# liuzl/rwkv-tts-rs

Measured on AMD Instinct MI355X. Metric: audio samples/sec (16 kHz) for RWKV-TTS 0.4B, batch=32 per GPU, higher is better.
Workload: dtype bf16; 1 GPU; config3: 32 requests/GPU, P=32 prompt, 32 global + 512 semantic tokens, exact sampler, + BiCodec vocoder -> PCM (vocoder of batch s overlapped with LM of batch s+1 on its own stream); global_batch=32, seq_len=577, parallelism=dp1 (request sharding)

## Files before the change

include/rwkvtts.h:

```cpp
#ifndef RWKVTTS_H
#define RWKVTTS_H

#include <stddef.h>
#include <stdint.h>

#ifdef __cplusplus
extern "C" {
#endif

#define RWKVTTS_EOS_TOKEN 8192
#define RWKVTTS_TAG_0 8193
#define RWKVTTS_TAG_1 8194
#define RWKVTTS_TAG_2 8195
#define RWKVTTS_GLOBAL_TOKEN_OFFSET 8196
#define RWKVTTS_SPECIAL_TOKEN_OFFSET 77823
#define RWKVTTS_N_GLOBAL 32
#define RWKVTTS_SEMANTIC_LIMIT 2048
#define RWKVTTS_HOP 320
#define RWKVTTS_SAMPLE_RATE 16000

#define RWKVTTS_OK 0
#define RWKVTTS_EINVAL -1
#define RWKVTTS_EHIP -2
#define RWKVTTS_ENOMEM -3
// ... 98 lines not shown
  int32_t token_chunk_size;
  int32_t use_graphs;
  int32_t wkv_variant;
  int32_t quant_layers;
  int32_t quant_type;
  uint32_t forms;
} rwkvtts_engine_desc;

#define RWKVTTS_FORM_SEPARATE_ATT 1u
#define RWKVTTS_FORM_SEPARATE_FFN 2u
#define RWKVTTS_FORM_LN_ROWS 4u
#define RWKVTTS_FORM_SLAB_HANDOFF 8u
#define RWKVTTS_FORM_SEPARATE_LNOUT 16u
#define RWKVTTS_FORM_SEPARATE_EMBED 32u
#define RWKVTTS_FORM_EXACT_SAMPLER 64u

#define RWKVTTS_QUANT_NONE 0
#define RWKVTTS_QUANT_INT8 1
#define RWKVTTS_QUANT_NF4 2
#define RWKVTTS_QUANT_SF4 3

int rwkvtts_engine_create(const rwkvtts_engine_desc* desc, const void* weights, size_t bytes,
                          int blob_on_device, rwkvtts_engine** out);
int rwkvtts_engine_destroy(rwkvtts_engine* e);
const char* rwkvtts_last_error(void);
int rwkvtts_engine_dims(const rwkvtts_engine* e, rwkvtts_dims* out);

int64_t rwkvtts_state_floats(const rwkvtts_engine* e);
int rwkvtts_slot_reset(rwkvtts_engine* e, int slot);
int rwkvtts_slot_read(rwkvtts_engine* e, int slot, float* host_out);
// ... 113 lines not shown
  int32_t persistent[RWKVTTS_MAX_ENGINES];
} rwkvtts_manager_stats;
int rwkvtts_manager_get_stats(rwkvtts_manager* m, rwkvtts_manager_stats* out);

typedef struct {
  int64_t steps;
  int64_t prefill_steps;
  double decode_ms;
  double prefill_ms;
  double sample_ms;
  int64_t decode_rows;
  int32_t profile_kernel_count;
  int32_t persistent;
} rwkvtts_stats;
int rwkvtts_get_stats(rwkvtts_engine* e, rwkvtts_stats* out);

int rwkvtts_set_profiling(rwkvtts_engine* e, int on);
int rwkvtts_profile_entry(rwkvtts_engine* e, int idx, char* name, int name_cap, int64_t* launches,
                          double* total_ms);

int rwkvtts_debug_advance(rwkvtts_engine* e, const float* logits, int n_rows, const void* rows, int exact,
                          int n_steps, int32_t* out_tok, int32_t* out_used, int32_t* out_phase);
int rwkvtts_debug_advance_ex(rwkvtts_engine* e, const float* logits, int n_rows, const void* rows, int exact,
                             int n_steps, int32_t* out_tok, int32_t* out_used, int32_t* out_phase);

typedef struct rwkvtts_codec rwkvtts_codec;
typedef struct {
  int32_t codebook_size;
  int32_t codebook_dim;
  int32_t latent_dim;
// ... 197 lines not shown
```

rwkv-tts-rs_amd/csrc/api.cpp:

```cpp
#include <string.h>

#include <mutex>
#include <new>

#include "engine.h"

namespace rwkvtts {
static thread_local std::string g_last_error;
void set_error(const std::string& msg) { g_last_error = msg; }
}

using namespace rwkvtts;

struct rwkvtts_engine {
  std::mutex mu;
  Engine eng;
};
#define LOCK(e) std::lock_guard<std::mutex> lock_((e)->mu)

#define GUARD(body)                                      \
  try {                                                  \
    body                                                 \
  } catch (const std::bad_alloc&) {                      \
    set_error("out of host memory");                     \
// ... 124 lines not shown
        results[i].n_global = results[i].n_semantic = 0;
      }
    return rc;
  })
}

int rwkvtts_get_stats(rwkvtts_engine* e, rwkvtts_stats* out) {
  RT_CHECK(e && out, RWKVTTS_EINVAL, "null argument");
  LOCK(e);
  *out = e->eng.stats;
  out->profile_kernel_count = (int32_t)e->eng.prof.size();
  out->persistent = e->eng.persistent() ? 1 : 0;
  return RWKVTTS_OK;
}

int rwkvtts_set_profiling(rwkvtts_engine* e, int on) {
  RT_CHECK(e, RWKVTTS_EINVAL, "null engine");
  RT_CHECK(on >= 0 && on <= 2, RWKVTTS_EINVAL, "set_profiling: 0, 1 or 2");
  LOCK(e);
  GUARD({
    e->eng.profiling = on == 1;
    return e->eng.set_graph_timing(on == 2);
  })
}

int rwkvtts_profile_entry(rwkvtts_engine* e, int idx, char* name, int name_cap, int64_t* launches,
                          double* total_ms) {
  RT_CHECK(e, RWKVTTS_EINVAL, "null engine");
  LOCK(e);
  RT_CHECK(idx >= 0 && idx < (int)e->eng.prof.size(), RWKVTTS_EINVAL, "profile index out of range");
// ... 12 lines not shown
```

rwkv-tts-rs_amd/csrc/engine.h:

```cpp
#pragma once
#include <map>
#include <string>
#include <vector>

#include "lm_kernels.h"
#include "sampler.h"
#include "sched.h"

namespace rwkvtts {

struct DebugAdvanceRow {
  int32_t mode;
  int32_t phase;
  int32_t top_k;
  int32_t fixed;
  int32_t n_sem;
  int32_t hard_min;
  int32_t win_bits;
  int32_t win_len;
  uint32_t key[8];
  uint64_t draw;
};
struct DebugAdvanceRowEx {
  DebugAdvanceRow row;
// ... 57 lines not shown
             rwkvtts_rng* const* rngs, int32_t* out, float* dbg_host = nullptr);
  int generate(const rwkvtts_request* reqs, int n, rwkvtts_result* res, const rwkvtts_token_sink* sinks = nullptr);
  int debug_advance(const float* logits, int n_rows, const struct DebugAdvanceRow* rows, int exact, int n_steps,
                    int32_t* out_tok, int32_t* out_used, int32_t* out_phase);
  int debug_advance_ex(const float* logits, int n_rows, const struct DebugAdvanceRowEx* rows, int exact, int n_steps,
                       int32_t* out_tok, int32_t* out_used, int32_t* out_phase);
  int serve(JobSource& src);
  bool validate(const rwkvtts_request& q, std::string& why) const { return rwkvtts::validate(q, dims.n_vocab, why); }
  int max_slots() const { return S_; }
  bool persistent() const { return att_persist_ || ffn_persist_; }
  bool take_recovered() {
    const bool r = recovered_;
    recovered_ = false;
    return r;
  }
  int64_t max_active = 0;
  int64_t admissions_ = 0;

  rwkvtts_dims dims{};
  rwkvtts_stats stats{};
  bool profiling = false;
  std::vector<ProfEntry> prof;
  int set_graph_timing(bool on);
  bool graph_timing() const { return d_gt_ != nullptr && gtime_; }

 private:
  int run_step(const StepPlan& p, bool upload);
  struct ServeState;
  struct Unit {
    bool valid = false, prefill = false, uploaded = false;
    int buf = 0;
  };
  int serve_loop(ServeState& st);
  int admit(ServeState& st, Job* j);
  int launch_unit(ServeState& st, Unit& u);
  int enqueue_snapshot(ServeState& st, const Unit& u);
  int finish_unit(const Unit& u, ServeState& st);
  int accumulate_stamps(const Unit& u);
  int launch_forward(int R, int n_seg, int n_lg, int head_rows, bool tok_from_ctrl, bool advance,
                     bool sampling_params = false);
  int upload_plan(const StepPlan& p);
  void prof_begin(hipEvent_t* ev);
  void prof_end(const char* name, hipEvent_t ev);
  int flush_prof();
  int dump_stamps();
  int reset_persistent();
  int degrade_persistent();
  static constexpr int64_t kDegradeWindow = 1024;
  int64_t units_ = 0;
// ... 80 lines not shown
      if ((int)tl_names_.size() > tl_n_) tl_names_.resize(tl_n_);
    }
    return RWKVTTS_OK;
  }
  static constexpr int kTlMax = 1024;
  bf16_t* wpack_ = nullptr;
  bf16_t* lora_pack_ = nullptr;
  const bf16_t* emb_ = nullptr;
  const bf16_t* head_ = nullptr;
  const float *ln0_w_ = nullptr, *ln0_b_ = nullptr, *lnout_w_ = nullptr, *lnout_b_ = nullptr;
  std::vector<LayerW> L_;
  float* wkv_ = nullptr;
  float* att_sh_ = nullptr;
  float* ffn_sh_ = nullptr;
  int* slot_par_ = nullptr;
  std::vector<int> par_host_;
  std::vector<SlotCtrl> ctrl_stage_;
  uint32_t* d_tok_ = nullptr;
  int4* d_rows_ = nullptr;
  int4* d_segs_ = nullptr;
  int* d_lg_rows_ = nullptr;
  int* d_lg_slot_ = nullptr;
  float *h0_ = nullptr, *h1_ = nullptr, *partA_ = nullptr, *partO_ = nullptr, *partF_ = nullptr,
        *partK_ = nullptr,
        *vfirst_ = nullptr, *logits_ = nullptr;
  bf16_t *xm_hi_ = nullptr, *xm_lo_ = nullptr, *z_hi_ = nullptr, *z_lo_ = nullptr,
         *xf_hi_ = nullptr, *xf_lo_ = nullptr, *xk_hi_ = nullptr, *xk_lo_ = nullptr,
         *xo_hi_ = nullptr, *xo_lo_ = nullptr;
  SlotCtrl* d_ctrl_ = nullptr;
  int32_t* d_sem_ = nullptr;
  SlotCtrl* h_ctrl_ = nullptr;
  int32_t* h_prog_ = nullptr;
// ... 28 lines not shown
```

rwkv-tts-rs_amd/csrc/engine.hip:

```cpp
#include "engine.h"

#include <fcntl.h>
#include <string.h>
#include <sys/file.h>
#include <unistd.h>

#include <algorithm>
#include <chrono>
#include <deque>
#include <map>
#include <mutex>
#include <random>

namespace rwkvtts {

template <typename T>
int Engine::alloc(T** p, size_t count) {
  void* q = nullptr;
  RT_HIP(hipMalloc(&q, std::max<size_t>(count * sizeof(T), 256)));
  RT_HIP(hipMemset(q, 0, std::max<size_t>(count * sizeof(T), 256)));
  allocs_.push_back(q);
  *p = (T*)q;
  return RWKVTTS_OK;
}
// ... 50 lines not shown
    if (*lock_fd >= 0) close(*lock_fd);
    *lock_fd = -1;
  }
}

Engine::~Engine() {
  release_persistent(device_, this, &lock_fd_);
  hipSetDevice(device_);
  if (stream_) hipStreamSynchronize(stream_);
  for (auto& g : graphs_) hipGraphExecDestroy(g.second);
  for (auto& e : pending_prof_) hipEventDestroy(e.second);
  for (void* p : allocs_) hipFree(p);
  for (void* p : {(void*)d_samp_logits_, (void*)d_keys_, (void*)d_draws_, (void*)d_out_, d_wide_})
    if (p) hipFree(p);
  if (h_ctrl_) hipHostFree(h_ctrl_);
  if (h_prog_) hipHostFree(h_prog_);
  if (h_gt_) hipHostFree(h_gt_);
  if (stream_) hipStreamDestroy(stream_);
}

#define RT_OK(x)                      \
  do {                                \
    int _r = (x);                     \
    if (_r != RWKVTTS_OK) return _r;  \
  } while (0)

int Engine::init(const rwkvtts_engine_desc& desc, const void* weights, size_t bytes, int on_device) {
  device_ = desc.device;
  RT_HIP(hipSetDevice(device_));
  {
// ... 32 lines not shown
  auto pick = [](int K, int want) {
    int ks = std::max(128, std::min(std::min(want, 512), K));
    while (ks > 128 && K % ks) ks >>= 1;
    return K / ks;
  };
  splitA_ = pick(C, 256);
  splitO_ = pick(C, 128);
  splitK_ = pick(C, 256);
  splitF_ = pick(F, 256);
  splitH_ = pick(C, 512);
  RT_CHECK(C % 128 == 0 && F % 128 == 0, RWKVTTS_EUNSUPPORTED, "K dims must be multiples of 128");
  RT_CHECK(splitA_ <= kMaxParts, RWKVTTS_EUNSUPPORTED, "n_embd too large for the WKV partial sum (raise kMaxParts)");
  state_perm_ = wkv_perm_layout(dims.d_decay, dims.d_aaa, dims.d_mv, dims.d_gate, splitA_, S_, desc.wkv_variant);
  constexpr uint32_t kKnownForms = RWKVTTS_FORM_SEPARATE_ATT | RWKVTTS_FORM_SEPARATE_FFN | RWKVTTS_FORM_LN_ROWS |
                                   RWKVTTS_FORM_SLAB_HANDOFF | RWKVTTS_FORM_SEPARATE_LNOUT |
                                   RWKVTTS_FORM_SEPARATE_EMBED | RWKVTTS_FORM_EXACT_SAMPLER;
  RT_CHECK((desc.forms & ~kKnownForms) == 0, RWKVTTS_EINVAL, "engine desc: unknown forms bits");
  att_persist_ = !(desc.forms & RWKVTTS_FORM_SEPARATE_ATT);
  ffn_persist_ = !(desc.forms & RWKVTTS_FORM_SEPARATE_FFN);
  fuse_ln1_ = !(desc.forms & RWKVTTS_FORM_LN_ROWS);
  gran_ = !(desc.forms & RWKVTTS_FORM_SLAB_HANDOFF);
  lnrow_ = !(desc.forms & RWKVTTS_FORM_SEPARATE_LNOUT);
  no_emb_fuse_ = (desc.forms & RWKVTTS_FORM_SEPARATE_EMBED) != 0;
  exact_sampler_ = (desc.forms & RWKVTTS_FORM_EXACT_SAMPLER) != 0;
  if ((ffn_persist_ || att_persist_) && !claim_persistent(desc.device, this, &lock_fd_)) ffn_persist_ = att_persist_ = false;
  if (const char* ds = getenv("RWKVTTS_DEBUG_STAMPS")) {
    std::string spec(ds);
    size_t pos = 0;
    while (pos < spec.size()) {
      size_t end = spec.find(';', pos);
      if (end == std::string::npos) end = spec.size();
      const std::string item = spec.substr(pos, end - pos);
      pos = end + 1;
      const size_t eq = item.find('=');
      if (eq == std::string::npos) continue;
      const std::string kind = item.substr(0, eq), path = item.substr(eq + 1);
      if (kind == "gemm") {
        dbg_gstamp_path_ = path;
        RT_OK(alloc(&dbg_gstamps_, 2 * 4096 * 4));
// ... 124 lines not shown
    for (int l = 0; l < dims.n_layer; ++l) {
      LayerW& w = L_[l];
      pack(w.wr, C, C, true); pack(w.wk, C, C, true); pack(w.wv, C, C, true);
      pack(w.w1t, Dw, C, true); pack(w.a1t, Da, C, true); pack(w.v1t, Dv, C, true); pack(w.g1t, Dg, C, true);
      pack(w.wo, C, C); pack(w.ffn_k, F, C); pack(w.ffn_v, C, F);
    }
    pack(head_, dims.n_vocab, C);
    RT_HIP(hipGetLastError());
  }
  RT_HIP(hipStreamSynchronize(stream_));
  const int64_t Lc = dims.n_layer;
  RT_OK(alloc(&wkv_, (size_t)S_ * Lc * H_ * 64 * 64));
  RT_OK(alloc(&att_sh_, (size_t)2 * S_ * Lc * C));
  RT_OK(alloc(&ffn_sh_, (size_t)2 * S_ * Lc * C));
  RT_OK(alloc(&slot_par_, (size_t)S_));
  par_host_.assign(S_, 0);
  ctrl_stage_.assign(S_, SlotCtrl{});
  RT_OK(alloc(&d_tok_, (size_t)Rmax_));
  RT_OK(alloc(&d_rows_, (size_t)Rmax_));
  RT_OK(alloc(&d_segs_, (size_t)std::max(Rmax_, S_)));
  RT_OK(alloc(&d_lg_rows_, (size_t)Rmax_));
  RT_OK(alloc(&d_lg_slot_, (size_t)Rmax_));
  const size_t RC = (size_t)Rmax_ * C;
  RT_OK(alloc(&h0_, RC));
  RT_OK(alloc(&h1_, RC));
  RT_OK(alloc(&xm_hi_, 6 * RC));
  RT_OK(alloc(&xm_lo_, 6 * RC));
  RT_OK(alloc(&partA_, (size_t)splitA_ * Rmax_ * ldA_));
  RT_OK(alloc(&z_hi_, RC));
  RT_OK(alloc(&z_lo_, RC));
  RT_OK(alloc(&partO_, (size_t)splitO_ * RC));
  RT_OK(alloc(&xf_hi_, RC));
// ... 31 lines not shown
    sync_bufs_.push_back({(int*)d_gran_, (size_t)ffn_gran_count(4, dims.n_ffn) * sizeof(uint64_t)});
    const int64_t ng = att_gran_count((int)dims.n_embd);
    RT_OK(alloc(&d_gran_att_, (size_t)ng));
    sync_bufs_.push_back({(int*)d_gran_att_, (size_t)ng * sizeof(uint64_t)});
  }

  RT_HIP(hipDeviceSynchronize());
  return RWKVTTS_OK;
}

int64_t Engine::state_floats() const {
  const int64_t C = dims.n_embd;
  return (int64_t)dims.n_layer * (2 * C + (int64_t)H_ * 64 * 64);
}

int Engine::slot_reset(int slot, bool sync) {
  RT_CHECK(slot >= 0 && slot < S_, RWKVTTS_EINVAL, "slot out of range");
  RT_HIP(hipSetDevice(device_));
  const int64_t C = dims.n_embd, Lc = dims.n_layer, per = Lc * H_ * 64 * 64;
  RT_HIP(hipMemsetAsync(wkv_ + slot * per, 0, per * 4, stream_));
  for (int p = 0; p < 2; ++p) {
    RT_HIP(hipMemsetAsync(att_sh_ + ((int64_t)p * S_ + slot) * Lc * C, 0, Lc * C * 4, stream_));
    RT_HIP(hipMemsetAsync(ffn_sh_ + ((int64_t)p * S_ + slot) * Lc * C, 0, Lc * C * 4, stream_));
  }
  par_host_[slot] = 0;
  RT_HIP(hipMemcpyAsync(slot_par_ + slot, &par_host_[slot], 4, hipMemcpyHostToDevice, stream_));
  if (sync) RT_HIP(hipStreamSynchronize(stream_));
  return RWKVTTS_OK;
}

static inline int64_t perm_index(int kind, int i, int j) {
  if (kind == 1) {
    const int t = 2 * i + (j >> 5), q = (j & 31) >> 2, e = j & 3;
    return ((int64_t)q * 128 + t) * 4 + e;
  }
  const int t = 4 * i + (j >> 4), q = (j & 15) >> 2, e = j & 3;
  return ((int64_t)q * 256 + t) * 4 + e;
}
void Engine::state_permute(const float* std_block, float* dev_block) {
  for (int i = 0; i < 64; ++i)
    for (int j = 0; j < 64; ++j) dev_block[perm_index(state_perm_, i, j)] = std_block[i * 64 + j];
}
// ... 15 lines not shown
    RT_HIP(hipMemcpy(o + C, wkv_ + ((int64_t)slot * Lc + l) * HNN, HNN * 4, hipMemcpyDeviceToHost));
    if (state_perm_) {
      std::vector<float> tmp(o + C, o + C + HNN);
      for (int h = 0; h < H_; ++h) state_unpermute(tmp.data() + (int64_t)h * 4096, o + C + (int64_t)h * 4096);
    }
    RT_HIP(hipMemcpy(o + C + HNN, ffn_sh_ + (((int64_t)par * S_ + slot) * Lc + l) * C, C * 4, hipMemcpyDeviceToHost));
  }
  return RWKVTTS_OK;
}

int Engine::slot_write(int slot, const float* in) {
  RT_CHECK(slot >= 0 && slot < S_, RWKVTTS_EINVAL, "slot out of range");
  RT_HIP(hipSetDevice(device_));
  RT_HIP(hipStreamSynchronize(stream_));
  const int64_t C = dims.n_embd, Lc = dims.n_layer, HNN = (int64_t)H_ * 64 * 64;
  par_host_[slot] = 0;
  RT_HIP(hipMemcpy(slot_par_ + slot, &par_host_[slot], 4, hipMemcpyHostToDevice));
  for (int64_t l = 0; l < Lc; ++l) {
    const float* o = in + l * (2 * C + HNN);
    RT_HIP(hipMemcpy(att_sh_ + (((int64_t)0 * S_ + slot) * Lc + l) * C, o, C * 4, hipMemcpyHostToDevice));
    if (state_perm_) {
      std::vector<float> tmp(HNN);
      for (int h = 0; h < H_; ++h) state_permute(o + C + (int64_t)h * 4096, tmp.data() + (int64_t)h * 4096);
      RT_HIP(hipMemcpy(wkv_ + ((int64_t)slot * Lc + l) * HNN, tmp.data(), HNN * 4, hipMemcpyHostToDevice));
    } else {
      RT_HIP(hipMemcpy(wkv_ + ((int64_t)slot * Lc + l) * HNN, o + C, HNN * 4, hipMemcpyHostToDevice));
    }
    RT_HIP(hipMemcpy(ffn_sh_ + (((int64_t)0 * S_ + slot) * Lc + l) * C, o + C + HNN, C * 4, hipMemcpyHostToDevice));
  }
  return RWKVTTS_OK;
}

// ... 705 lines not shown
int Engine::generate(const rwkvtts_request* reqs, int n, rwkvtts_result* res, const rwkvtts_token_sink* sinks) {
  stats = rwkvtts_stats{};
  max_active = 0;
  ListSource src(reqs, n, res, sinks);
  const int rc = serve(src);
  if (rc != RWKVTTS_OK && sinks) src.fail_rest(rc);
  return rc;
}

struct Engine::ServeState {
  explicit ServeState(JobSource& s) : src(s) {}
  JobSource& src;
  std::vector<Active> act;
  std::vector<int> free_slots;
  std::vector<Job*> fresh;
  bool open = true;
  Unit pending;
  StepPlan dp;
  bool dp_valid = false;
  UnitEvents ev;
  std::random_device rd;
};

int Engine::admit(ServeState& st, Job* j) {
  const rwkvtts_request& q = j->req;
  j->res->status = 0;
  j->res->n_global = j->res->n_semantic = 0;
  std::string why;
  if (!validate(q, why)) {
    set_error("request rejected: " + why);
// ... 12 lines not shown
                         hipHostMallocDefault));
  if (const char* fa = getenv("RWKVTTS_TEST_FAIL_ADMIT")) {
    if (++admissions_ == atoi(fa)) {
      set_error("injected admission failure (RWKVTTS_TEST_FAIL_ADMIT)");
      return RWKVTTS_EHIP;
    }
  }
  Admission ad = admission_of(q, q.has_seed ? 0 : (((uint64_t)st.rd() << 32) ^ st.rd()));
  const int slot = st.free_slots.back();
  st.free_slots.pop_back();
  rwkvtts_rng rg, rs;
  rwkvtts_rng_seed_from_u64(ad.gseed, &rg);
  rwkvtts_rng_seed_from_u64(ad.sseed, &rs);
  memcpy(ad.ctrl.gkey, rg.key, 32);
  memcpy(ad.ctrl.skey, rs.key, 32);
  RT_OK(slot_reset(slot, false));
  ctrl_stage_[slot] = ad.ctrl;
  RT_HIP(hipMemcpyAsync(d_ctrl_ + slot, &ctrl_stage_[slot], sizeof(SlotCtrl), hipMemcpyHostToDevice, stream_));
  Active a;
  a.job = j;
  a.slot = slot;
  a.sink = sink_of(j);
  a.zero_shot = ad.zero_shot;
  a.pinned = ad.pinned;
  a.own_sampling = ad.own_sampling;
  a.prompt = std::move(ad.prompt);
  a.total = ad.total;
  st.act.push_back(std::move(a));
  st.dp_valid = false;
  return RWKVTTS_OK;
}

int Engine::launch_unit(ServeState& st, Unit& u) {
  std::vector<Active>& act = st.act;
  u.valid = true;
  u.uploaded = false;
  u.prefill = std::any_of(act.begin(), act.end(), [](const Active& a) { return a.in_prompt(); });
  u.buf = st.pending.valid ? st.pending.buf ^ 1 : 0;
  RT_HIP(hipEventRecord(st.ev.ev0[u.buf], stream_));
  if (u.prefill) {
    RT_OK(run_step(mixed_plan(act, chunk_, dims.n_vocab), true));
    st.dp_valid = false;
    stats.prefill_steps++;
    return RWKVTTS_OK;
  }
  if (!st.dp_valid) {
    st.dp = decode_plan(act);
    RT_OK(upload_plan(st.dp));
    st.dp_valid = u.uploaded = true;
  }
  const int K = window_len(act, kLookahead, profiling || d_tl_);
  if (d_tl_) RT_HIP(hipMemsetAsync(d_tl_, 0, (size_t)kTlStride * kTlMax * 8, stream_));
  for (int k = 0; k < K; ++k) {
    st.dp.head_rows = head_rows_of(act, dims.n_vocab);
    RT_OK(run_step(st.dp, false));
    for (auto& a : act) a.advances++;
// ... 68 lines not shown
    while ((q = hipEventQuery(st.ev.ev1[b])) == hipErrorNotReady) __builtin_ia32_pause();
    RT_HIP(q);
  }
  float ms = 0;
  hipEventElapsedTime(&ms, st.ev.ev0[b], st.ev.ev1[b]);
  (u.prefill ? stats.prefill_ms : stats.decode_ms) += ms;
  RT_OK(flush_prof());
  RT_OK(accumulate_stamps(u));
  ++units_;
  const SlotCtrl* snap = h_ctrl_ + (size_t)b * (S_ + 1);
  if (const int code = *(const int*)(snap + S_)) {
    persist_fault_ = code;
    set_error("persistent decode launch: a hand-off wait timed out (code " + std::to_string(code) + ")");
    return RWKVTTS_EHIP;
  }
  auto retiring = [&](const Active& a) { return !a.in_prompt() && snap[a.slot].phase == kPhDone; };
  bool copied = false;
  for (auto& a : act) {
    const SlotCtrl& c = snap[a.slot];
    if (!retiring(a) || !a.job->res->semantic_tokens || c.n_sem <= 0) continue;
    RT_HIP(hipMemcpyAsync(a.job->res->semantic_tokens, d_sem_ + (int64_t)a.slot * RWKVTTS_SEMANTIC_LIMIT,
                          sizeof(int32_t) * c.n_sem, hipMemcpyDeviceToHost, stream_));
    copied = true;
  }
  if (copied) RT_HIP(hipStreamSynchronize(stream_));
  for (auto& a : act) {
    if (!a.sink || a.in_prompt()) continue;
    const SlotCtrl& c = snap[a.slot];
    const bool done = c.phase == kPhDone;
    const int n = std::min(c.n_sem, a.copied_hi[b]);
// ... 22 lines not shown
    st.free_slots.push_back(act[i].slot);
    act.erase(act.begin() + i);
  }
  if (act.size() != st.dp.rows.size()) st.dp_valid = false;
  return RWKVTTS_OK;
}

int Engine::serve_loop(ServeState& st) {
  while (true) {
    if (st.open && !st.free_slots.empty()) {
      st.open = st.src.next((int)st.free_slots.size(), st.act.empty(), st.fresh);
      while (!st.fresh.empty()) {
        RT_OK(admit(st, st.fresh.front()));
        st.fresh.erase(st.fresh.begin());
      }
    }
    if (st.act.empty()) {
      if (!st.open) return RWKVTTS_OK;
      continue;
    }
    std::sort(st.act.begin(), st.act.end(), [](const Active& x, const Active& y) { return x.slot < y.slot; });
    Unit now;
    RT_OK(launch_unit(st, now));
    RT_OK(enqueue_snapshot(st, now));
    if (st.pending.valid) {
      const Unit old = st.pending;
      st.pending.valid = false;
      RT_OK(finish_unit(old, st));
    }
    const bool can_admit = st.open && !st.free_slots.empty();
// ... 15 lines not shown
    const int code = persist_fault_;
    persist_fault_ = 0;
    const bool degrade = last_fault_unit_ >= 0 && units_ - last_fault_unit_ <= kDegradeWindow;
    last_fault_unit_ = units_;
    recovered_ = reset_persistent() == RWKVTTS_OK && (!degrade || degrade_persistent() == RWKVTTS_OK);
    if (recovered_ && d_drop_ && test_drops_left_ > 0) {
      --test_drops_left_;
      const int one = 1;
      recovered_ = hipMemcpy(d_drop_, &one, sizeof(int), hipMemcpyHostToDevice) == hipSuccess;
    }
    set_error("persistent decode launch: a hand-off wait timed out (code " + std::to_string(code) +
              "); the unit's requests failed, the engine was reset" +
              (degrade ? " and now runs the separate launches (second timeout)" : ""));
  }
  if (rc != RWKVTTS_OK) {
    for (Job* j : st.fresh) fail_job(src, j, rc, 0);
    for (auto& a : st.act) fail_job(src, a.job, rc, a.sink ? a.delivered : -1);
    return rc;
  }
  return dump_stamps();
}

int Engine::reset_persistent() {
  RT_HIP(hipSetDevice(device_));
  RT_HIP(hipMemsetAsync(d_ctrl_ + S_, 0, sizeof(SlotCtrl), stream_));
  for (auto& b : sync_bufs_) RT_HIP(hipMemsetAsync(b.first, 0, b.second, stream_));
  if (d_epoch_) {
    int ep = 0;
    RT_HIP(hipMemcpyAsync(&ep, d_epoch_, sizeof(int), hipMemcpyDeviceToHost, stream_));
    RT_HIP(hipStreamSynchronize(stream_));
// ... 77 lines not shown
```

rwkv-tts-rs_amd/csrc/sched.h:

```cpp
#pragma once
#include <math.h>
#include <stdint.h>
#include <string.h>

#include <algorithm>
#include <string>
#include <vector>

#include "../../include/rwkvtts.h"
#include "slot_ctrl.h"

namespace rwkvtts {

struct Job;

struct alignas(16) Int4 {
  int32_t x, y, z, w;
};

struct StepPlan {
  std::vector<uint32_t> tok;
  std::vector<Int4> rows;
  std::vector<Int4> segs;
  std::vector<int> lg_rows;
// ... 5 lines not shown
};

struct Active {
  Job* job = nullptr;
  int slot = 0;
  std::vector<uint32_t> prompt;
  int prefilled = 0;
  int advances = 0;
  int total = 0;
  bool zero_shot = false;
  bool pinned = false;
  bool own_sampling = false;
  const rwkvtts_token_sink* sink = nullptr;
  int delivered = 0;
  int copied_hi[2] = {0, 0};
  bool in_prompt() const { return prefilled < (int)prompt.size(); }
};

inline bool is_zero_shot(const rwkvtts_request& q) { return q.ref_global != nullptr && q.ref_semantic != nullptr; }
inline bool is_pinned(const rwkvtts_request& q) { return q.pinned_voice != 0; }

inline bool validate(const rwkvtts_request& q, int n_vocab, std::string& why) {
  auto ids_ok = [&](const int32_t* p, int n, int lo, int hi, const char* what) {
    if (n < 0 || (n > 0 && !p)) {
      why = std::string(what) + ": bad array";
      return false;
    }
    for (int i = 0; i < n; ++i)
      if (p[i] < lo || p[i] >= hi) {
        why = std::string(what) + ": id " + std::to_string(p[i]) + " out of range";
// ... 124 lines not shown
    c.phase = kPhSemantic;
    for (int i = 0; i < RWKVTTS_N_GLOBAL; ++i) {
      a.prompt.push_back((uint32_t)(q.ref_global[i] + RWKVTTS_GLOBAL_TOKEN_OFFSET));
      c.global_out[c.n_global++] = q.ref_global[i];
    }
    a.prompt.push_back(RWKVTTS_TAG_1);
    a.total = c.sem_limit;
  } else {
    c.mode = 0;
    c.phase = kPhGlobal;
    a.total = RWKVTTS_N_GLOBAL + 1 + c.sem_limit;
  }
  return a;
}

inline void append_decode_row(StepPlan& p, int slot) {
  const int r = (int)p.rows.size();
  p.rows.push_back({slot, kRowFirst | kRowLast | kRowCtrl, -1, 0});
  if (!p.tok_from_ctrl) p.tok.push_back(0);
  p.segs.push_back({slot, r, 1, 0});
  p.lg_rows.push_back(r);
  p.lg_slot.push_back(slot);
}

enum LogitRows { kLogitsNone, kLogitsLast, kLogitsAll };

inline void append_token_rows(StepPlan& p, int slot, const uint32_t* tok, int take, LogitRows lg) {
  const int r0 = (int)p.rows.size();
  for (int t = 0; t < take; ++t) {
    const int flags = (t == 0 ? kRowFirst : 0) | (t == take - 1 ? kRowLast : 0);
// ... 13 lines not shown
    if (!a.in_prompt()) all_global &= !a.zero_shot && !a.pinned && a.advances <= RWKVTTS_N_GLOBAL;
  return std::min(all_global ? 4096 : 8193, n_vocab);
}

inline StepPlan mixed_plan(std::vector<Active>& act, int chunk, int n_vocab) {
  StepPlan p;
  p.advance = true;
  int budget = chunk;
  for (const Active& a : act) {
    if (a.in_prompt()) continue;
    append_decode_row(p, a.slot);
    --budget;
  }
  budget = std::max(budget, 1);
  for (Active& a : act) {
    const int left = (int)a.prompt.size() - a.prefilled;
    if (left <= 0 || budget <= 0) continue;
    const int take = std::min(left, budget);
    append_token_rows(p, a.slot, a.prompt.data() + a.prefilled, take, take == left ? kLogitsLast : kLogitsNone);
    a.prefilled += take;
    budget -= take;
  }
  p.head_rows = head_rows_of(act, n_vocab);
  p.sampling_params = any_own_sampling(act);
  for (Active& a : act) a.advances += !a.in_prompt();
  return p;
}

inline StepPlan decode_plan(const std::vector<Active>& act) {
  StepPlan p;
  p.tok_from_ctrl = true;
  p.advance = true;
  p.sampling_params = any_own_sampling(act);
  for (const Active& a : act) append_decode_row(p, a.slot);
  return p;
}

inline int window_len(const std::vector<Active>& act, int lookahead, bool single) {
  int K = single ? 1 : lookahead;
  for (const Active& a : act) K = std::min(K, std::max(1, a.total - a.advances));
// ... 19 lines not shown
```

rwkv-tts-rs_amd/rwkvtts/_ffi.py:

```python
import ctypes
import os

_HERE = os.path.dirname(os.path.abspath(__file__))
LIB_PATH = os.environ.get("RWKVTTS_LIB") or os.path.join(_HERE, "librwkvtts.so")


def build_id() -> str:
    import glob
    import hashlib
    csrc = os.path.join(_HERE, "..", "csrc")
    inc = os.path.join(_HERE, "..", "..", "include")
    files = sorted(glob.glob(os.path.join(csrc, "*.hip")) + glob.glob(os.path.join(csrc, "*.cpp")) +
                   glob.glob(os.path.join(csrc, "*.h")) + [os.path.join(csrc, "Makefile")] +
                   glob.glob(os.path.join(inc, "*.h")), key=os.path.basename)
    h = hashlib.sha256()
    for f in files:
        h.update(os.path.basename(f).encode())
        with open(f, "rb") as fh:
            h.update(fh.read())
    return h.hexdigest()[:16]

EOS_TOKEN = 8192
TAG_0, TAG_1, TAG_2 = 8193, 8194, 8195
GLOBAL_TOKEN_OFFSET = 8196
# ... 11 lines not shown

class Dims(ctypes.Structure):
    _fields_ = [(n, ctypes.c_int32) for n in (
        "n_layer", "n_embd", "head_size", "n_ffn", "n_vocab", "d_decay", "d_aaa", "d_mv", "d_gate")]


class EngineDesc(ctypes.Structure):
    _fields_ = [("device", ctypes.c_int32), ("max_slots", ctypes.c_int32),
                ("token_chunk_size", ctypes.c_int32), ("use_graphs", ctypes.c_int32),
                ("wkv_variant", ctypes.c_int32), ("quant_layers", ctypes.c_int32),
                ("quant_type", ctypes.c_int32), ("forms", ctypes.c_uint32)]


FORM_SEPARATE_ATT, FORM_SEPARATE_FFN, FORM_LN_ROWS, FORM_SLAB_HANDOFF = 1, 2, 4, 8
FORM_SEPARATE_LNOUT, FORM_SEPARATE_EMBED, FORM_EXACT_SAMPLER = 16, 32, 64
CODEC_WEIGHTS_AUTO, CODEC_WEIGHTS_BF16, CODEC_WEIGHTS_HILO = 0, 1, 2
CODEC_FORM_SEPARATE_RESUNIT, CODEC_FORM_CHANNEL_LAST = 1, 2


QUANT_NONE, QUANT_INT8, QUANT_NF4, QUANT_SF4 = 0, 1, 2, 3


class Input(ctypes.Structure):
    _fields_ = [("slot", ctypes.c_int32), ("tokens", ctypes.POINTER(ctypes.c_uint32)),
                ("n_tokens", ctypes.c_int32), ("option", ctypes.c_int32)]


class Rng(ctypes.Structure):
    _fields_ = [("key", ctypes.c_uint32 * 8), ("draw_index", ctypes.c_uint64)]

# ... 23 lines not shown
                ("sampling_set", ctypes.c_int32), ("global_sampling", PhaseSampling),
                ("semantic_sampling", PhaseSampling), ("pinned_voice", ctypes.c_int32)]


class Result(ctypes.Structure):
    _fields_ = [("status", ctypes.c_int32), ("n_global", ctypes.c_int32),
                ("n_semantic", ctypes.c_int32), ("global_tokens", ctypes.c_int32 * N_GLOBAL),
                ("semantic_tokens", ctypes.POINTER(ctypes.c_int32))]


class Stats(ctypes.Structure):
    _fields_ = [("steps", ctypes.c_int64), ("prefill_steps", ctypes.c_int64),
                ("decode_ms", ctypes.c_double), ("prefill_ms", ctypes.c_double),
                ("sample_ms", ctypes.c_double), ("decode_rows", ctypes.c_int64),
                ("profile_kernel_count", ctypes.c_int32), ("persistent", ctypes.c_int32)]


class ManagerDesc(ctypes.Structure):
    _fields_ = [("n_engines", ctypes.c_int32), ("devices", ctypes.c_int32 * MAX_ENGINES),
                ("engine", EngineDesc), ("max_batch_size", ctypes.c_int32),
                ("collect_timeout_ms", ctypes.c_int32)]


class ManagerStats(ctypes.Structure):
    _fields_ = [("submitted", ctypes.c_int64), ("completed", ctypes.c_int64), ("batches", ctypes.c_int64),
                ("served", ctypes.c_int64 * MAX_ENGINES), ("max_active", ctypes.c_int64 * MAX_ENGINES),
                ("steps", ctypes.c_int64 * MAX_ENGINES), ("bcast_ranks", ctypes.c_int32),
                ("bcast_rccl", ctypes.c_int32), ("bcast_ms", ctypes.c_double),
                ("waiters", ctypes.c_int32), ("reserved", ctypes.c_int32),
                ("persistent", ctypes.c_int32 * MAX_ENGINES)]
# ... 101 lines not shown
                                                     ctypes.POINTER(ctypes.c_uint64)]),
    "rwkvtts_manager_wait_tokens": (ctypes.c_int, [ctypes.c_void_p, ctypes.c_uint64, ctypes.c_int32, ctypes.c_int,
                                                   ctypes.c_void_p, ctypes.POINTER(ctypes.c_int32), ctypes.c_void_p,
                                                   ctypes.POINTER(ctypes.c_int32), ctypes.POINTER(ctypes.c_int32),
                                                   ctypes.POINTER(ctypes.c_int32)]),
    "rwkvtts_manager_create": (ctypes.c_int, [ctypes.POINTER(ManagerDesc), ctypes.c_void_p, ctypes.c_size_t,
                                              ctypes.POINTER(ctypes.c_void_p)]),
    "rwkvtts_manager_destroy": (ctypes.c_int, [ctypes.c_void_p]),
    "rwkvtts_manager_submit": (ctypes.c_int, [ctypes.c_void_p, ctypes.POINTER(Request),
                                              ctypes.POINTER(ctypes.c_uint64)]),
    "rwkvtts_manager_wait": (ctypes.c_int, [ctypes.c_void_p, ctypes.c_uint64, ctypes.c_int, ctypes.POINTER(Result)]),
    "rwkvtts_manager_generate_batch": (ctypes.c_int, [ctypes.c_void_p, ctypes.POINTER(Request), ctypes.c_int,
                                                      ctypes.POINTER(Result)]),
    "rwkvtts_manager_get_stats": (ctypes.c_int, [ctypes.c_void_p, ctypes.POINTER(ManagerStats)]),
    "rwkvtts_get_stats": (ctypes.c_int, [ctypes.c_void_p, ctypes.POINTER(Stats)]),
    "rwkvtts_set_profiling": (ctypes.c_int, [ctypes.c_void_p, ctypes.c_int]),
    "rwkvtts_debug_advance": (ctypes.c_int, [ctypes.c_void_p, ctypes.c_void_p, ctypes.c_int, ctypes.c_void_p,
                                             ctypes.c_int, ctypes.c_int, ctypes.c_void_p, ctypes.c_void_p,
                                             ctypes.c_void_p]),
    "rwkvtts_debug_advance_ex": (ctypes.c_int, [ctypes.c_void_p, ctypes.c_void_p, ctypes.c_int, ctypes.c_void_p,
                                                ctypes.c_int, ctypes.c_int, ctypes.c_void_p, ctypes.c_void_p,
                                                ctypes.c_void_p]),
    "rwkvtts_profile_entry": (ctypes.c_int, [ctypes.c_void_p, ctypes.c_int, ctypes.c_char_p, ctypes.c_int,
                                             ctypes.POINTER(ctypes.c_int64), ctypes.POINTER(ctypes.c_double)]),
    "rwkvtts_codec_blob_bytes": (ctypes.c_int64, [ctypes.POINTER(CodecDims)]),
    "rwkvtts_codec_synth_weights": (ctypes.c_int, [ctypes.POINTER(CodecDims), ctypes.c_uint64, ctypes.c_void_p]),
    "rwkvtts_codec_create": (ctypes.c_int, [ctypes.c_int, ctypes.POINTER(CodecDims), ctypes.c_void_p,
                                            ctypes.POINTER(ctypes.c_void_p)]),
    "rwkvtts_codec_create_ex": (ctypes.c_int, [ctypes.c_int, ctypes.POINTER(CodecDims), ctypes.c_void_p,
                                               ctypes.c_int, ctypes.POINTER(ctypes.c_void_p)]),
# ... 101 lines not shown
```

rwkv-tts-rs_amd/rwkvtts/runtime.py:

```python
import ctypes
import dataclasses
import threading
from typing import List, Optional, Sequence

import numpy as np

from . import _ffi
from ._ffi import check, lib


class StdRng:

    def __init__(self, rng_struct):
        self._s = rng_struct

    @classmethod
    def seed_from_u64(cls, seed: int) -> "StdRng":
        s = _ffi.Rng()
        lib().rwkvtts_rng_seed_from_u64(ctypes.c_uint64(seed & 0xFFFFFFFFFFFFFFFF), ctypes.byref(s))
        return cls(s)

    @property
    def key(self):
        return list(self._s.key)
# ... 265 lines not shown
                sinks[i].fn = fns[-1]
        rc = lib().rwkvtts_generate_batch_stream(self._h, reqs, n, res, sinks)
        if raised:
            raise raised[0]
        check(rc, "generate_batch_stream")
        out, self.last_status = _unpack_results(res, sem_bufs)
        return out

    @_locked
    def stats(self):
        s = _ffi.Stats()
        check(lib().rwkvtts_get_stats(self._h, ctypes.byref(s)), "get_stats")
        return {f: getattr(s, f) for f, _ in _ffi.Stats._fields_}

    @_locked
    def set_profiling(self, on):
        mode = on if isinstance(on, int) and not isinstance(on, bool) else (1 if on else 0)
        check(lib().rwkvtts_set_profiling(self._h, mode), "set_profiling")

    @_locked
    def profile(self):
        out = {}
        n = self.stats()["profile_kernel_count"]
        for i in range(n):
            name = ctypes.create_string_buffer(64)
            la = ctypes.c_int64()
            ms = ctypes.c_double()
            check(lib().rwkvtts_profile_entry(self._h, i, name, 64, ctypes.byref(la), ctypes.byref(ms)), "profile_entry")
            out[name.value.decode()] = (int(la.value), float(ms.value))
        return out
# ... 246 lines not shown
```

Before: 11.12 million samples/s.

## Add prompt prefix state cache and batched slot admission kernel

Adds an 8-entry cache of recurrent state keyed on the property-token prefix of each request. A hit restores the WKV and shift state in a single admission kernel and skips prefilling those tokens. A miss makes the request build the entry, with the prefill split so the state can be snapshotted at the prefix boundary and then published. Per-slot memsets and control copies are replaced by one batched k_admit launch per admission round. The trade-off is an extra tail prefill step and publish copies on misses, plus device memory for the cache entries.

Result: slower. 10.99 million samples/s (-1.2%).

```diff
diff --git a/include/rwkvtts.h b/include/rwkvtts.h
--- a/include/rwkvtts.h
+++ b/include/rwkvtts.h
@@ -136,6 +136,7 @@
 #define RWKVTTS_FORM_SEPARATE_LNOUT 16u
 #define RWKVTTS_FORM_SEPARATE_EMBED 32u
 #define RWKVTTS_FORM_EXACT_SAMPLER 64u
+#define RWKVTTS_FORM_NO_PREFIX_CACHE 128u
 
 #define RWKVTTS_QUANT_NONE 0
 #define RWKVTTS_QUANT_INT8 1
@@ -279,6 +280,14 @@
   int32_t persistent;
 } rwkvtts_stats;
 int rwkvtts_get_stats(rwkvtts_engine* e, rwkvtts_stats* out);
+
+typedef struct {
+  int64_t lookups;
+  int64_t hits;
+  int64_t builds;
+  int64_t evictions;
+} rwkvtts_prefix_cache_stats;
+int rwkvtts_get_prefix_cache_stats(rwkvtts_engine* e, rwkvtts_prefix_cache_stats* out);
 
 int rwkvtts_set_profiling(rwkvtts_engine* e, int on);
 int rwkvtts_profile_entry(rwkvtts_engine* e, int idx, char* name, int name_cap, int64_t* launches,
diff --git a/rwkv-tts-rs_amd/csrc/api.cpp b/rwkv-tts-rs_amd/csrc/api.cpp
--- a/rwkv-tts-rs_amd/csrc/api.cpp
+++ b/rwkv-tts-rs_amd/csrc/api.cpp
@@ -162,6 +162,14 @@
   return RWKVTTS_OK;
 }
 
+int rwkvtts_get_prefix_cache_stats(rwkvtts_engine* e, rwkvtts_prefix_cache_stats* out) {
+  RT_CHECK(e && out, RWKVTTS_EINVAL, "null argument");
+  LOCK(e);
+  const PrefixTable& t = e->eng.prefix_table();
+  *out = rwkvtts_prefix_cache_stats{t.lookups, t.hits, t.builds, t.evictions};
+  return RWKVTTS_OK;
+}
+
 int rwkvtts_set_profiling(rwkvtts_engine* e, int on) {
   RT_CHECK(e, RWKVTTS_EINVAL, "null engine");
   RT_CHECK(on >= 0 && on <= 2, RWKVTTS_EINVAL, "set_profiling: 0, 1 or 2");
diff --git a/rwkv-tts-rs_amd/csrc/engine.h b/rwkv-tts-rs_amd/csrc/engine.h
--- a/rwkv-tts-rs_amd/csrc/engine.h
+++ b/rwkv-tts-rs_amd/csrc/engine.h
@@ -95,6 +95,7 @@
     recovered_ = false;
     return r;
   }
+  const PrefixTable& prefix_table() const { return ptab_; }
   int64_t max_active = 0;
   int64_t admissions_ = 0;
 
@@ -114,6 +115,10 @@
   };
   int serve_loop(ServeState& st);
   int admit(ServeState& st, Job* j);
+  int launch_admit(const int* slots, const int* entry, int n, bool with_ctrl);
+  int flush_admissions(ServeState& st);
+  int enqueue_publish(const Active& a);
+  void abandon_claims(ServeState& st);
   int launch_unit(ServeState& st, Unit& u);
   int enqueue_snapshot(ServeState& st, const Unit& u);
   int finish_unit(const Unit& u, ServeState& st);
@@ -224,8 +229,11 @@
   float* att_sh_ = nullptr;
   float* ffn_sh_ = nullptr;
   int* slot_par_ = nullptr;
-  std::vector<int> par_host_;
-  std::vector<SlotCtrl> ctrl_stage_;
+  SlotCtrl* ctrl_stage_ = nullptr;
+  bool prefix_cache_ = true;
+  PrefixTable ptab_;
+  float* pstore_[kPrefixEntries] = {};
+  int64_t prefix_entry_floats() const { return (int64_t)dims.n_layer * (2 * dims.n_embd + (int64_t)H_ * 64 * 64) + 4; }
   uint32_t* d_tok_ = nullptr;
   int4* d_rows_ = nullptr;
   int4* d_segs_ = nullptr;
diff --git a/rwkv-tts-rs_amd/csrc/engine.hip b/rwkv-tts-rs_amd/csrc/engine.hip
--- a/rwkv-tts-rs_amd/csrc/engine.hip
+++ b/rwkv-tts-rs_amd/csrc/engine.hip
@@ -88,6 +88,7 @@
   for (void* p : {(void*)d_samp_logits_, (void*)d_keys_, (void*)d_draws_, (void*)d_out_, d_wide_})
     if (p) hipFree(p);
   if (h_ctrl_) hipHostFree(h_ctrl_);
+  if (ctrl_stage_) hipHostFree(ctrl_stage_);
   if (h_prog_) hipHostFree(h_prog_);
   if (h_gt_) hipHostFree(h_gt_);
   if (stream_) hipStreamDestroy(stream_);
@@ -150,7 +151,8 @@
   state_perm_ = wkv_perm_layout(dims.d_decay, dims.d_aaa, dims.d_mv, dims.d_gate, splitA_, S_, desc.wkv_variant);
   constexpr uint32_t kKnownForms = RWKVTTS_FORM_SEPARATE_ATT | RWKVTTS_FORM_SEPARATE_FFN | RWKVTTS_FORM_LN_ROWS |
                                    RWKVTTS_FORM_SLAB_HANDOFF | RWKVTTS_FORM_SEPARATE_LNOUT |
-                                   RWKVTTS_FORM_SEPARATE_EMBED | RWKVTTS_FORM_EXACT_SAMPLER;
+                                   RWKVTTS_FORM_SEPARATE_EMBED | RWKVTTS_FORM_EXACT_SAMPLER |
+                                   RWKVTTS_FORM_NO_PREFIX_CACHE;
   RT_CHECK((desc.forms & ~kKnownForms) == 0, RWKVTTS_EINVAL, "engine desc: unknown forms bits");
   att_persist_ = !(desc.forms & RWKVTTS_FORM_SEPARATE_ATT);
   ffn_persist_ = !(desc.forms & RWKVTTS_FORM_SEPARATE_FFN);
@@ -159,6 +161,7 @@
   lnrow_ = !(desc.forms & RWKVTTS_FORM_SEPARATE_LNOUT);
   no_emb_fuse_ = (desc.forms & RWKVTTS_FORM_SEPARATE_EMBED) != 0;
   exact_sampler_ = (desc.forms & RWKVTTS_FORM_EXACT_SAMPLER) != 0;
+  prefix_cache_ = !(desc.forms & RWKVTTS_FORM_NO_PREFIX_CACHE);
   if ((ffn_persist_ || att_persist_) && !claim_persistent(desc.device, this, &lock_fd_)) ffn_persist_ = att_persist_ = false;
   if (const char* ds = getenv("RWKVTTS_DEBUG_STAMPS")) {
     std::string spec(ds);
@@ -313,8 +316,8 @@
   RT_OK(alloc(&att_sh_, (size_t)2 * S_ * Lc * C));
   RT_OK(alloc(&ffn_sh_, (size_t)2 * S_ * Lc * C));
   RT_OK(alloc(&slot_par_, (size_t)S_));
-  par_host_.assign(S_, 0);
-  ctrl_stage_.assign(S_, SlotCtrl{});
+  RT_HIP(hipHostMalloc((void**)&ctrl_stage_, sizeof(SlotCtrl) * (size_t)S_, hipHostMallocDefault));
+  memset(ctrl_stage_, 0, sizeof(SlotCtrl) * (size_t)S_);
   RT_OK(alloc(&d_tok_, (size_t)Rmax_));
   RT_OK(alloc(&d_rows_, (size_t)Rmax_));
   RT_OK(alloc(&d_segs_, (size_t)std::max(Rmax_, S_)));
@@ -376,18 +379,114 @@
   return (int64_t)dims.n_layer * (2 * C + (int64_t)H_ * 64 * 64);
 }
 
+constexpr int kAdmitMax = 32;
+struct AdmitArgs {
+  float *wkv, *att_sh, *ffn_sh;
+  int* slot_par;
+  SlotCtrl* ctrl;
+  const SlotCtrl* stage;
+  const float* store[kPrefixEntries];
+  int64_t wkv4, sh4;
+  int S, n, with_ctrl;
+  int16_t slot[kAdmitMax];
+  int8_t entry[kAdmitMax];
+};
+__global__ __launch_bounds__(256) void k_admit(const AdmitArgs a) {
+  const int slot = a.slot[blockIdx.y];
+  const int ent = a.entry[blockIdx.y];
+  const float4* src = ent >= 0 ? (const float4*)a.store[ent] : nullptr;
+  const int64_t wkv4 = a.wkv4, sh4 = a.sh4, total = wkv4 + 4 * sh4;
+  const int par = src ? (*(const int*)(src + wkv4 + 2 * sh4) & 1) : 0;
+  const float4 zero = {0.f, 0.f, 0.f, 0.f};
+  for (int64_t j = (int64_t)blockIdx.x * 256 + threadIdx.x; j < total; j += (int64_t)gridDim.x * 256) {
+    float4* dst;
+    float4 v = zero;
+    if (j < wkv4) {
+      dst = (float4*)a.wkv + (int64_t)slot * wkv4 + j;
+      if (src) v = src[j];
+    } else {
+      const int64_t k = j - wkv4;
+      const int plane = k < 2 * sh4 ? (k < sh4 ? 0 : 1) : (k < 3 * sh4 ? 2 : 3);
+      const int64_t c = k - plane * sh4;
+      const int p = plane & 1, ffn = plane >> 1;
+      dst = (float4*)(ffn ? a.ffn_sh : a.att_sh) + ((int64_t)p * a.S + slot) * sh4 + c;
+      if (src && p == par) v = src[wkv4 + (ffn ? sh4 : 0) + c];
+    }
+    *dst = v;
+  }
+  if (blockIdx.x == 0) {
+    if (threadIdx.x == 0) a.slot_par[slot] = par;
+    if (a.with_ctrl) {
+      const int* s = (const int*)(a.stage + slot);
+      int* d = (int*)(a.ctrl + slot);
+      for (int t = threadIdx.x; t < (int)(sizeof(SlotCtrl) / 4); t += 256) d[t] = s[t];
+    }
+  }
+}
+__global__ __launch_bounds__(256) void k_prefix_publish(const float* wkv, const float* att_sh, const float* ffn_sh,
+                                                        const int* slot_par, float* entry, int64_t wkv4, int64_t sh4,
+                                                        int S, int slot) {
+  const int par = slot_par[slot] & 1;
+  const int64_t total = wkv4 + 2 * sh4;
+  float4* dst = (float4*)entry;
+  for (int64_t j = (int64_t)blockIdx.x * 256 + threadIdx.x; j < total; j += (int64_t)gridDim.x * 256) {
+    if (j < wkv4) {
+      dst[j] = ((const float4*)wkv)[(int64_t)slot * wkv4 + j];
+    } else {
+      const int64_t k = j - wkv4;
+      const int ffn = k >= sh4;
+      dst[j] = ((const float4*)(ffn ? ffn_sh : att_sh))[((int64_t)par * S + slot) * sh4 + (k - ffn * sh4)];
+    }
+  }
+  if (blockIdx.x == 0 && threadIdx.x == 0) *(int4*)(dst + total) = make_int4(par, 0, 0, 0);
+}
+static int admit_grid(int64_t n4) { return (int)std::min<int64_t>(2048, std::max<int64_t>(1, (n4 + 256 * 8 - 1) / (256 * 8))); }
+
+int Engine::launch_admit(const int* slots, const int* entry, int n, bool with_ctrl) {
+  const int64_t C = dims.n_embd, Lc = dims.n_layer;
+  RT_CHECK((Lc * C) % 4 == 0, RWKVTTS_EINVAL, "admission: n_layer * n_embd must be a multiple of 4");
+  for (int o = 0; o < n; o += kAdmitMax) {
+    AdmitArgs a{};
+    a.wkv = wkv_;
+    a.att_sh = att_sh_;
+    a.ffn_sh = ffn_sh_;
+    a.slot_par = slot_par_;
+    a.ctrl = d_ctrl_;
+    a.stage = ctrl_stage_;
+    for (int i = 0; i < kPrefixEntries; ++i) a.store[i] = pstore_[i];
+    a.wkv4 = Lc * H_ * 64 * 64 / 4;
+    a.sh4 = Lc * C / 4;
+    a.S = S_;
+    a.n = std::min(kAdmitMax, n - o);
+    a.with_ctrl = with_ctrl ? 1 : 0;
+    for (int i = 0; i < a.n; ++i) {
+      const int slot = slots[o + i], e = entry ? entry[o + i] : -1;
+      RT_CHECK(slot >= 0 && slot < S_ && e >= -1 && e < kPrefixEntries && (e < 0 || pstore_[e]), RWKVTTS_EINVAL,
+               "admission: slot or cache entry out of range");
+      a.slot[i] = (int16_t)slot;
+      a.entry[i] = (int8_t)e;
+    }
+    hipLaunchKernelGGL(k_admit, dim3(admit_grid(a.wkv4 + 4 * a.sh4), a.n), dim3(256), 0, stream_, a);
+  }
+  RT_HIP(hipGetLastError());
+  return RWKVTTS_OK;
+}
+
 int Engine::slot_reset(int slot, bool sync) {
   RT_CHECK(slot >= 0 && slot < S_, RWKVTTS_EINVAL, "slot out of range");
   RT_HIP(hipSetDevice(device_));
-  const int64_t C = dims.n_embd, Lc = dims.n_layer, per = Lc * H_ * 64 * 64;
-  RT_HIP(hipMemsetAsync(wkv_ + slot * per, 0, per * 4, stream_));
-  for (int p = 0; p < 2; ++p) {
-    RT_HIP(hipMemsetAsync(att_sh_ + ((int64_t)p * S_ + slot) * Lc * C, 0, Lc * C * 4, stream_));
-    RT_HIP(hipMemsetAsync(ffn_sh_ + ((int64_t)p * S_ + slot) * Lc * C, 0, Lc * C * 4, stream_));
-  }
-  par_host_[slot] = 0;
-  RT_HIP(hipMemcpyAsync(slot_par_ + slot, &par_host_[slot], 4, hipMemcpyHostToDevice, stream_));
+  RT_OK(launch_admit(&slot, nullptr, 1, false));
   if (sync) RT_HIP(hipStreamSynchronize(stream_));
+  return RWKVTTS_OK;
+}
+
+int Engine::enqueue_publish(const Active& a) {
+  const int64_t C = dims.n_embd, Lc = dims.n_layer, wkv4 = Lc * H_ * 64 * 64 / 4, sh4 = Lc * C / 4;
+  RT_CHECK(a.build_entry >= 0 && a.build_entry < kPrefixEntries && pstore_[a.build_entry], RWKVTTS_EINVAL,
+           "prefix cache: publish without an entry");
+  hipLaunchKernelGGL(k_prefix_publish, dim3(admit_grid(wkv4 + 2 * sh4)), dim3(256), 0, stream_, wkv_, att_sh_, ffn_sh_,
+                     slot_par_, pstore_[a.build_entry], wkv4, sh4, S_, a.slot);
+  RT_HIP(hipGetLastError());
   return RWKVTTS_OK;
 }
 
@@ -433,8 +532,8 @@
   RT_HIP(hipSetDevice(device_));
   RT_HIP(hipStreamSynchronize(stream_));
   const int64_t C = dims.n_embd, Lc = dims.n_layer, HNN = (int64_t)H_ * 64 * 64;
-  par_host_[slot] = 0;
-  RT_HIP(hipMemcpy(slot_par_ + slot, &par_host_[slot], 4, hipMemcpyHostToDevice));
+  const int par0 = 0;
+  RT_HIP(hipMemcpy(slot_par_ + slot, &par0, 4, hipMemcpyHostToDevice));
   for (int64_t l = 0; l < Lc; ++l) {
     const float* o = in + l * (2 * C + HNN);
     RT_HIP(hipMemcpy(att_sh_ + (((int64_t)0 * S_ + slot) * Lc + l) * C, o, C * 4, hipMemcpyHostToDevice));
@@ -1170,6 +1269,7 @@
   std::vector<Active> act;
   std::vector<int> free_slots;
   std::vector<Job*> fresh;
+  std::vector<int> adm_slots, adm_entry;
   bool open = true;
   Unit pending;
   StepPlan dp;
@@ -1212,10 +1312,30 @@
   rwkvtts_rng_seed_from_u64(ad.sseed, &rs);
   memcpy(ad.ctrl.gkey, rg.key, 32);
   memcpy(ad.ctrl.skey, rs.key, 32);
-  RT_OK(slot_reset(slot, false));
   ctrl_stage_[slot] = ad.ctrl;
-  RT_HIP(hipMemcpyAsync(d_ctrl_ + slot, &ctrl_stage_[slot], sizeof(SlotCtrl), hipMemcpyHostToDevice, stream_));
   Active a;
+  int hit = -1;
+  if (const int plen = prefix_cache_ ? prefix_len_of(q) : 0) {
+    hit = prefix_lookup(ptab_, ad.prompt.data(), plen);
+    if (hit >= 0) {
+      a.prefilled = plen;
+    } else {
+      const int e = prefix_claim(ptab_, ad.prompt.data(), plen, slot);
+      if (e >= 0 && !pstore_[e]) {
+        const hipError_t me = hipMalloc((void**)&pstore_[e], sizeof(float) * (size_t)prefix_entry_floats());
+        if (me != hipSuccess) {
+          prefix_abandon(ptab_, e);
+          pstore_[e] = nullptr;
+          RT_HIP(me);
+        }
+        allocs_.push_back(pstore_[e]);
+      }
+      a.build_entry = e;
+    }
+    a.prefix_len = plen;
+  }
+  st.adm_slots.push_back(slot);
+  st.adm_entry.push_back(hit);
   a.job = j;
   a.slot = slot;
   a.sink = sink_of(j);
@@ -1229,6 +1349,22 @@
   return RWKVTTS_OK;
 }
 
+int Engine::flush_admissions(ServeState& st) {
+  if (st.adm_slots.empty()) return RWKVTTS_OK;
+  const int rc = launch_admit(st.adm_slots.data(), st.adm_entry.data(), (int)st.adm_slots.size(), true);
+  st.adm_slots.clear();
+  st.adm_entry.clear();
+  return rc;
+}
+
+void Engine::abandon_claims(ServeState& st) {
+  for (Active& a : st.act) {
+    if (a.build_entry >= 0) prefix_abandon(ptab_, a.build_entry);
+    a.build_entry = -1;
+    a.publish_pending = false;
+  }
+}
+
 int Engine::launch_unit(ServeState& st, Unit& u) {
   std::vector<Active>& act = st.act;
   u.valid = true;
@@ -1237,7 +1373,15 @@
   u.buf = st.pending.valid ? st.pending.buf ^ 1 : 0;
   RT_HIP(hipEventRecord(st.ev.ev0[u.buf], stream_));
   if (u.prefill) {
-    RT_OK(run_step(mixed_plan(act, chunk_, dims.n_vocab), true));
+    const StepPlan mp = mixed_plan(act, chunk_, dims.n_vocab);
+    RT_OK(run_step(mp, true));
+    for (Active& a : act)
+      if (a.build_entry >= 0 && !a.publish_pending && a.prefilled == a.prefix_len) {
+        RT_OK(enqueue_publish(a));
+        a.publish_pending = true;
+      }
+    const StepPlan tail = builder_tail_plan(act, mp, dims.n_vocab);
+    if (!tail.rows.empty()) RT_OK(run_step(tail, true));
     st.dp_valid = false;
     stats.prefill_steps++;
     return RWKVTTS_OK;
@@ -1336,6 +1480,12 @@
     set_error("persistent decode launch: a hand-off wait timed out (code " + std::to_string(code) + ")");
     return RWKVTTS_EHIP;
   }
+  for (Active& a : act)
+    if (u.prefill && a.publish_pending) {
+      prefix_publish(ptab_, a.build_entry);
+      a.build_entry = -1;
+      a.publish_pending = false;
+    }
   auto retiring = [&](const Active& a) { return !a.in_prompt() && snap[a.slot].phase == kPhDone; };
   bool copied = false;
   for (auto& a : act) {
@@ -1388,6 +1538,7 @@
         RT_OK(admit(st, st.fresh.front()));
         st.fresh.erase(st.fresh.begin());
       }
+      RT_OK(flush_admissions(st));
     }
     if (st.act.empty()) {
       if (!st.open) return RWKVTTS_OK;
@@ -1433,6 +1584,7 @@
               (degrade ? " and now runs the separate launches (second timeout)" : ""));
   }
   if (rc != RWKVTTS_OK) {
+    abandon_claims(st);
     for (Job* j : st.fresh) fail_job(src, j, rc, 0);
     for (auto& a : st.act) fail_job(src, a.job, rc, a.sink ? a.delivered : -1);
     return rc;
diff --git a/rwkv-tts-rs_amd/csrc/sched.h b/rwkv-tts-rs_amd/csrc/sched.h
--- a/rwkv-tts-rs_amd/csrc/sched.h
+++ b/rwkv-tts-rs_amd/csrc/sched.h
@@ -43,6 +43,11 @@
   const rwkvtts_token_sink* sink = nullptr;
   int delivered = 0;
   int copied_hi[2] = {0, 0};
+  int prefix_len = 0;
+  int build_entry = -1;
+  bool publish_pending = false;
+  int deferred = 0;
+  bool builder() const { return build_entry >= 0 && prefilled < prefix_len; }
   bool in_prompt() const { return prefilled < (int)prompt.size(); }
 };
 
@@ -197,6 +202,73 @@
   return a;
 }
 
+constexpr int kPrefixCap = 16;
+constexpr int kPrefixEntries = 8;
+
+inline int prefix_len_of(const rwkvtts_request& q) {
+  if (q.n_property <= 0 || q.n_property + 1 > kPrefixCap) return 0;
+  return q.n_property + 1;
+}
+
+struct PrefixEntry {
+  enum State : int { kEmpty, kBuilding, kValid };
+  State state = kEmpty;
+  int builder_slot = -1;
+  int len = 0;
+  uint32_t key[kPrefixCap] = {};
+  uint64_t used = 0;
+};
+struct PrefixTable {
+  PrefixEntry e[kPrefixEntries];
+  uint64_t clock = 0;
+  int64_t lookups = 0, hits = 0, builds = 0, evictions = 0;
+};
+
+inline int prefix_find(const PrefixTable& t, const uint32_t* key, int len) {
+  for (int i = 0; i < kPrefixEntries; ++i) {
+    const PrefixEntry& e = t.e[i];
+    if (e.state != PrefixEntry::kEmpty && e.len == len && memcmp(e.key, key, sizeof(uint32_t) * (size_t)len) == 0) return i;
+  }
+  return -1;
+}
+inline int prefix_lookup(PrefixTable& t, const uint32_t* key, int len) {
+  ++t.lookups;
+  const int i = prefix_find(t, key, len);
+  if (i < 0 || t.e[i].state != PrefixEntry::kValid) return -1;
+  ++t.hits;
+  t.e[i].used = ++t.clock;
+  return i;
+}
+inline int prefix_claim(PrefixTable& t, const uint32_t* key, int len, int slot) {
+  if (len <= 0 || len > kPrefixCap || prefix_find(t, key, len) >= 0) return -1;
+  int pick = -1;
+  for (int i = 0; i < kPrefixEntries && pick < 0; ++i)
+    if (t.e[i].state == PrefixEntry::kEmpty) pick = i;
+  if (pick < 0) {
+    for (int i = 0; i < kPrefixEntries; ++i)
+      if (t.e[i].state == PrefixEntry::kValid && (pick < 0 || t.e[i].used < t.e[pick].used)) pick = i;
+    if (pick < 0) return -1;
+    ++t.evictions;
+  }
+  PrefixEntry& e = t.e[pick];
+  e.state = PrefixEntry::kBuilding;
+  e.builder_slot = slot;
+  e.len = len;
+  memcpy(e.key, key, sizeof(uint32_t) * (size_t)len);
+  e.used = ++t.clock;
+  return pick;
+}
+inline void prefix_publish(PrefixTable& t, int i) {
+  if (i < 0 || i >= kPrefixEntries || t.e[i].state != PrefixEntry::kBuilding) return;
+  t.e[i].state = PrefixEntry::kValid;
+  t.e[i].builder_slot = -1;
+  ++t.builds;
+}
+inline void prefix_abandon(PrefixTable& t, int i) {
+  if (i < 0 || i >= kPrefixEntries || t.e[i].state != PrefixEntry::kBuilding) return;
+  t.e[i] = PrefixEntry{};
+}
+
 inline void append_decode_row(StepPlan& p, int slot) {
   const int r = (int)p.rows.size();
   p.rows.push_back({slot, kRowFirst | kRowLast | kRowCtrl, -1, 0});
@@ -240,16 +312,37 @@
   }
   budget = std::max(budget, 1);
   for (Active& a : act) {
+    a.deferred = 0;
     const int left = (int)a.prompt.size() - a.prefilled;
     if (left <= 0 || budget <= 0) continue;
     const int take = std::min(left, budget);
-    append_token_rows(p, a.slot, a.prompt.data() + a.prefilled, take, take == left ? kLogitsLast : kLogitsNone);
-    a.prefilled += take;
+    const int now = a.builder() ? std::min(take, a.prefix_len - a.prefilled) : take;
+    a.deferred = take - now;
+    append_token_rows(p, a.slot, a.prompt.data() + a.prefilled, now, now == left ? kLogitsLast : kLogitsNone);
+    a.prefilled += now;
     budget -= take;
   }
   p.head_rows = head_rows_of(act, n_vocab);
   p.sampling_params = any_own_sampling(act);
   for (Active& a : act) a.advances += !a.in_prompt();
+  return p;
+}
+
+inline StepPlan builder_tail_plan(std::vector<Active>& act, const StepPlan& main, int n_vocab) {
+  StepPlan p;
+  p.advance = true;
+  p.sampling_params = main.sampling_params;
+  bool all_global = true;
+  for (Active& a : act) {
+    if (a.deferred <= 0) continue;
+    const int left = (int)a.prompt.size() - a.prefilled, take = std::min(a.deferred, left);
+    append_token_rows(p, a.slot, a.prompt.data() + a.prefilled, take, take == left ? kLogitsLast : kLogitsNone);
+    a.prefilled += take;
+    a.deferred = 0;
+    if (!a.in_prompt()) all_global &= !a.zero_shot && !a.pinned && a.advances <= RWKVTTS_N_GLOBAL;
+    a.advances += !a.in_prompt();
+  }
+  p.head_rows = std::max(main.head_rows, std::min(all_global ? 4096 : 8193, n_vocab));
   return p;
 }
 
diff --git a/rwkv-tts-rs_amd/rwkvtts/_ffi.py b/rwkv-tts-rs_amd/rwkvtts/_ffi.py
--- a/rwkv-tts-rs_amd/rwkvtts/_ffi.py
+++ b/rwkv-tts-rs_amd/rwkvtts/_ffi.py
@@ -49,6 +49,7 @@
 
 FORM_SEPARATE_ATT, FORM_SEPARATE_FFN, FORM_LN_ROWS, FORM_SLAB_HANDOFF = 1, 2, 4, 8
 FORM_SEPARATE_LNOUT, FORM_SEPARATE_EMBED, FORM_EXACT_SAMPLER = 16, 32, 64
+FORM_NO_PREFIX_CACHE = 128
 CODEC_WEIGHTS_AUTO, CODEC_WEIGHTS_BF16, CODEC_WEIGHTS_HILO = 0, 1, 2
 CODEC_FORM_SEPARATE_RESUNIT, CODEC_FORM_CHANNEL_LAST = 1, 2
 
@@ -102,6 +103,11 @@
                 ("decode_ms", ctypes.c_double), ("prefill_ms", ctypes.c_double),
                 ("sample_ms", ctypes.c_double), ("decode_rows", ctypes.c_int64),
                 ("profile_kernel_count", ctypes.c_int32), ("persistent", ctypes.c_int32)]
+
+
+class PrefixCacheStats(ctypes.Structure):
+    _fields_ = [("lookups", ctypes.c_int64), ("hits", ctypes.c_int64),
+                ("builds", ctypes.c_int64), ("evictions", ctypes.c_int64)]
 
 
 class ManagerDesc(ctypes.Structure):
@@ -233,6 +239,7 @@
                                                       ctypes.POINTER(Result)]),
     "rwkvtts_manager_get_stats": (ctypes.c_int, [ctypes.c_void_p, ctypes.POINTER(ManagerStats)]),
     "rwkvtts_get_stats": (ctypes.c_int, [ctypes.c_void_p, ctypes.POINTER(Stats)]),
+    "rwkvtts_get_prefix_cache_stats": (ctypes.c_int, [ctypes.c_void_p, ctypes.POINTER(PrefixCacheStats)]),
     "rwkvtts_set_profiling": (ctypes.c_int, [ctypes.c_void_p, ctypes.c_int]),
     "rwkvtts_debug_advance": (ctypes.c_int, [ctypes.c_void_p, ctypes.c_void_p, ctypes.c_int, ctypes.c_void_p,
                                              ctypes.c_int, ctypes.c_int, ctypes.c_void_p, ctypes.c_void_p,
diff --git a/rwkv-tts-rs_amd/rwkvtts/runtime.py b/rwkv-tts-rs_amd/rwkvtts/runtime.py
--- a/rwkv-tts-rs_amd/rwkvtts/runtime.py
+++ b/rwkv-tts-rs_amd/rwkvtts/runtime.py
@@ -303,6 +303,12 @@
         return {f: getattr(s, f) for f, _ in _ffi.Stats._fields_}
 
     @_locked
+    def prefix_cache_stats(self):
+        s = _ffi.PrefixCacheStats()
+        check(lib().rwkvtts_get_prefix_cache_stats(self._h, ctypes.byref(s)), "get_prefix_cache_stats")
+        return {f: getattr(s, f) for f, _ in _ffi.PrefixCacheStats._fields_}
+
+    @_locked
     def set_profiling(self, on):
         mode = on if isinstance(on, int) and not isinstance(on, bool) else (1 if on else 0)
         check(lib().rwkvtts_set_profiling(self._h, mode), "set_profiling")
```
